# Dimev/grail-rs

Hardware: AMD Instinct MI355X
Metric: audio samples/sec (whole node) at 48 kHz, batch=65536 utterances (higher is better)
Workload: dtype f32

## Files before the change

### grail-rs_amd/csrc/api_internal.hpp

```cpp
#pragma once

#include <dlfcn.h>
#include <hip/hip_runtime.h>
#include <rccl/rccl.h>

#include <algorithm>
#include <atomic>
#include <cmath>
#include <condition_variable>
#include <cstdio>
#include <deque>
#include <map>
#include <mutex>
#include <thread>
#include <cstdlib>
#include <cstring>
#include <new>
#include <string>
#include <unordered_map>
#include <vector>

#include "../../include/grail_hip.h"
#include "kernels.h"

struct PlanCache;

#ifdef GRAIL_FAST_PROF
constexpr size_t TRUNCATED_WORDS = 8 + 64;
#else
constexpr size_t TRUNCATED_WORDS = 4;
#endif

struct grail_ctx {
    int device = 0;
    int cus = 256;
    int device_cus = 256;
    hipStream_t stream = nullptr;
    hipEvent_t ev_start = nullptr, ev_stop = nullptr;
    bool have_timing = false;
    std::vector<grail_voice> voices;
    grail::DevVoice *d_voices = nullptr;
    float *d_voice_elems = nullptr;
    struct VoiceInfo {
        bool upper_silent = false, live4_ok = false, scan_ok = false, split_ok = false;
        uint32_t warmup = 0;
    };
    std::vector<VoiceInfo> voice_info;
    bool voices_upper_silent = false;
    bool voices_live4_ok = false;
    bool voices_scan_ok = false;
    int scan_debug = 0;
    int sort_option = 1;
    int64_t pipe8_max_groups = -1;
    int64_t pipe4_max_groups = -1;
    int scan_option = 1;
    int64_t scan_max_utts = -1;
    int64_t scan_split_max = -1;
    int ragged_option = 1;
    int pipe_spread = 1;
    int two_waves_option = 1;
    int packed_option = 1;
    int composite_option = 1;
    int row_groups_option = 1;
    double voices_sharpness = INFINITY;
    std::vector<double> voice_sharpness;
    int64_t fast_limit = (int64_t)GRAIL_FAST_SHARPNESS_LIMIT;
    int mid_option = 1;
    int64_t mid_limit = (int64_t)GRAIL_FAST_SHARPNESS_LIMIT_EXACT_COEFFICIENTS;
    bool voices_split_ok = false;
    uint32_t max_warmup = 0;
    float max_rate = 0.0f;
    int split_option = 1;
    int64_t split_chunks = 0;
    int64_t split_span = 0;
    int64_t split_ff_permille = 165;
    int64_t split_min_utts = -1;
    int last_split = 0;
    int last_fast = 0;
    int last_blocks = 0;
    float max_dt = 0.0f;
    float max_pitch_jitter = 0.0f;
    int last_formants = 8, last_lanes = 0, last_pipe = 0;
    int last_packed = 0;
    uint32_t *d_truncated = nullptr;
    uint64_t slow_steps = 0;
    uint64_t fast_tiles = 0, general_steps = 0;
    uint32_t seen_counters[4] = {0, 0, 0, 0};
    int lanes_option = 0;
    int skip_silent_option = 1;
    int pipeline_option = 1;
    int pipe_round32 = 1;
    uint64_t voices_epoch = 0;
    uint64_t options_epoch = 0;
    int fast_option = 0;
    std::string last_kernel = "none";
    ncclComm_t comm = nullptr;
    uint32_t comm_rank = 0, comm_world = 1;
    void *host_pipe = nullptr;
    void *mix_state = nullptr;
};

struct grail_stream {
    const grail_batch *batch = nullptr;
    uint32_t *d_state = nullptr;
    uint64_t lanes = 0;
    int L = 1;
    bool started = false;
    bool live4 = false, half_capable = false, any_blend = false;
    uint64_t voices_epoch = 0;
    grail_batch *own = nullptr;
    uint32_t ring_cap = 0;
    uint32_t *d_counts = nullptr;
    uint32_t *d_open = nullptr;
    uint32_t *d_consumed = nullptr;
    std::vector<uint32_t> appended;
    std::vector<uint32_t> consumed;
    std::vector<uint8_t> open;
    std::vector<grail_synthesis_elem> last_elem;
    std::vector<uint8_t> last_has;
    grail::DevSeg *d_new = nullptr;
// ... 151 lines not shown
```

### grail-rs_amd/csrc/grail_api.cpp

```cpp
#include "api_internal.hpp"

using namespace grail;
using namespace grail::host;

static_assert(sizeof(grail_synthesis_elem) == 196, "SynthesisElem is 49 x f32");
static_assert(sizeof(grail_phoneme_elem) == sizeof(DevSeg), "PhonemeElem uploads as-is");
static_assert(offsetof(grail_phoneme_elem, phoneme) == offsetof(DevSeg, elem), "layout");
static_assert(offsetof(grail_phoneme_elem, frequency) == offsetof(DevSeg, frequency), "layout");
static_assert(sizeof(grail_voice) == 4 + 2 * 196 + 5 * 4, "Voice layout");
static_assert(GRAIL_UNIQUE_ID_BYTES == NCCL_UNIQUE_ID_BYTES, "unique id size");

namespace grail {
namespace host {

namespace {
thread_local std::string g_last_error;
std::atomic<uint64_t> g_epoch{0};
}

std::string &last_error() { return g_last_error; }

int fail(int status, const std::string &msg)
{
    g_last_error = msg;
// ... 426 lines not shown
        return GRAIL_OK;
    }
    if (std::strcmp(name, "skip_silent_formants") == 0) {
        ctx->skip_silent_option = value ? 1 : 0;
        return GRAIL_OK;
    }
    if (std::strcmp(name, "small_batch_pipeline") == 0) {
        ctx->pipeline_option = value ? 1 : 0;
        return GRAIL_OK;
    }
    if (std::strcmp(name, "arithmetic") == 0) {
        if (value != 0 && value != 1 && value != 2)
            return fail(GRAIL_ERR_INVALID_ARG, "arithmetic must be 0 (exact), 1 (fast) or 2 (fast, exact coefficients)");
        ctx->fast_option = (int)value;
        return GRAIL_OK;
    }
    if (std::strcmp(name, "fast_exact_coefficients") == 0) {
        ctx->mid_option = value ? 1 : 0;
        return GRAIL_OK;
    }
    if (std::strcmp(name, "fast_sharpness_limit_exact_coefficients") == 0) {
        if (value < 0) return fail(GRAIL_ERR_INVALID_ARG, "negative limit");
        ctx->mid_limit = value;
        return GRAIL_OK;
    }
    if (std::strcmp(name, "time_parallel_scan") == 0) {
        ctx->scan_option = value ? 1 : 0;
        return GRAIL_OK;
    }
    if (std::strcmp(name, "packed_launch_order") == 0) {
        ctx->packed_option = value ? 1 : 0;
        return GRAIL_OK;
    }
    if (std::strcmp(name, "sort_by_length") == 0) {
        ctx->sort_option = value ? 1 : 0;
        return GRAIL_OK;
    }
    if (std::strcmp(name, "time_split") == 0) {
        ctx->split_option = value ? 1 : 0;
        return GRAIL_OK;
    }
    if (std::strcmp(name, "time_split_chunks") == 0) {
        if (value < 0 || value > SPLIT_MAX_CHUNKS) return fail(GRAIL_ERR_INVALID_ARG, "time_split_chunks must be 0 (auto) .. 64");
        ctx->split_chunks = value;
        return GRAIL_OK;
    }
    if (std::strcmp(name, "time_split_span_samples") == 0) {
        if (value < 0 || value > 0x7fffffff) return fail(GRAIL_ERR_INVALID_ARG, "time_split_span_samples out of range");
        ctx->split_span = value;
        return GRAIL_OK;
    }
    if (std::strcmp(name, "time_split_ff_cost_permille") == 0) {
        if (value < 0 || value > 1000) return fail(GRAIL_ERR_INVALID_ARG, "time_split_ff_cost_permille must be 0 .. 1000");
        ctx->split_ff_permille = value;
        return GRAIL_OK;
    }
    if (std::strcmp(name, "time_split_min_utterances") == 0) {
        if (value < -1) return fail(GRAIL_ERR_INVALID_ARG, "negative limit");
        ctx->split_min_utts = value;
        return GRAIL_OK;
    }
    if (std::strcmp(name, "fast_sharpness_limit") == 0) {
        if (value < 0) return fail(GRAIL_ERR_INVALID_ARG, "negative limit");
        ctx->fast_limit = value;
        return GRAIL_OK;
    }
// ... 90 lines not shown
        *value = ctx->composite_option;
        return GRAIL_OK;
    }
    if (std::strcmp(name, "row_groups") == 0) {
        *value = ctx->row_groups_option;
        return GRAIL_OK;
    }
    if (std::strcmp(name, "ragged_plan") == 0) {
        *value = ctx->ragged_option;
        return GRAIL_OK;
    }
    if (std::strcmp(name, "two_waves_per_simd") == 0) {
        *value = ctx->two_waves_option;
        return GRAIL_OK;
    }
    if (std::strcmp(name, "pipeline_spread") == 0) {
        *value = ctx->pipe_spread;
        return GRAIL_OK;
    }
    if (std::strcmp(name, "pipeline4_max_groups") == 0) {
        *value = ctx->pipe4_max_groups;
        return GRAIL_OK;
    }
    if (std::strcmp(name, "pipeline8_max_groups") == 0) {
        *value = ctx->pipe8_max_groups;
        return GRAIL_OK;
    }
    if (std::strcmp(name, "pipeline_round32") == 0) {
        *value = ctx->pipe_round32;
        return GRAIL_OK;
    }
    if (std::strcmp(name, "packed_launch_order") == 0) {
        *value = ctx->packed_option;
        return GRAIL_OK;
    }
    if (std::strcmp(name, "last_launch_packed") == 0) {
        *value = ctx->last_packed;
        return GRAIL_OK;
    }
    if (std::strcmp(name, "sort_by_length") == 0) {
        *value = ctx->sort_option;
        return GRAIL_OK;
    }
    if (std::strcmp(name, "last_launch_fast") == 0) {
        *value = ctx->last_fast;
        return GRAIL_OK;
    }
    if (std::strcmp(name, "last_launch_blocks") == 0) {
        *value = ctx->last_blocks;
        return GRAIL_OK;
    }
    if (std::strcmp(name, "time_split") == 0) {
        *value = ctx->split_option;
        return GRAIL_OK;
    }
    if (std::strcmp(name, "time_split_chunks") == 0) {
        *value = ctx->split_chunks;
        return GRAIL_OK;
    }
    if (std::strcmp(name, "time_split_span_samples") == 0) {
        *value = ctx->split_span;
        return GRAIL_OK;
    }
    if (std::strcmp(name, "time_split_ff_cost_permille") == 0) {
        *value = ctx->split_ff_permille;
        return GRAIL_OK;
// ... 266 lines not shown
int grail_batch_lengths(grail_ctx *ctx, const grail_batch *batch, uint32_t max_len,
                        uint32_t *out_len)
{
    int rc = bind(ctx);
    if (rc) return rc;
    if ((rc = check_ready(ctx, batch))) return rc;
    if (!out_len && batch->n_utt) return fail(GRAIL_ERR_INVALID_ARG, "out_len is NULL");
    if (batch->n_utt == 0) return GRAIL_OK;
    uint32_t *d_len = nullptr;
    HIP_TRY(hipMalloc((void **)&d_len, (size_t)batch->n_utt * sizeof(uint32_t)));
    LenArgs a{};
    a.segs = batch->d_segs;
    a.seg_offsets = batch->d_offsets;
    a.voice_ids = batch->d_voice_ids;
    a.voices = ctx->d_voices;
    a.out_len = d_len;
    a.n_utt = batch->n_utt;
    a.n_voices = (uint32_t)ctx->voices.size();
    a.max_len = max_len;
    hipError_t e = launch_lengths(a, ctx->stream);
    if (e == hipSuccess)
        e = hipMemcpyAsync(out_len, d_len, (size_t)batch->n_utt * sizeof(uint32_t),
                           hipMemcpyDeviceToHost, ctx->stream);
    if (e == hipSuccess) e = hipStreamSynchronize(ctx->stream);
    (void)hipFree(d_len);
    if (e != hipSuccess) return hip_fail(e, "grail_batch_lengths");
    return GRAIL_OK;
}

int grail_sync(grail_ctx *ctx)
{
    int rc = bind(ctx);
    if (rc) return rc;
    uint32_t flags[4] = {0, 0, 0, 0};
    HIP_TRY(hipMemcpyAsync(flags, ctx->d_truncated, sizeof flags, hipMemcpyDeviceToHost, ctx->stream));
    HIP_TRY(hipStreamSynchronize(ctx->stream));
    const uint32_t flag = flags[0];
    ctx->slow_steps += (uint32_t)(flags[1] - ctx->seen_counters[1]);
    ctx->fast_tiles += (uint32_t)(flags[2] - ctx->seen_counters[2]);
    ctx->general_steps += (uint32_t)(flags[3] - ctx->seen_counters[3]);
    for (int i = 1; i < 4; ++i) ctx->seen_counters[i] = flags[i];
    if (flag) {
        HIP_TRY(hipMemsetAsync(ctx->d_truncated, 0, sizeof(uint32_t), ctx->stream));
        HIP_TRY(hipStreamSynchronize(ctx->stream));
    }
    if (flag) {
        return fail(GRAIL_ERR_BUFFER_TOO_SMALL,
                    "at least one utterance did not end within out_stride samples");
    }
    return GRAIL_OK;
}

const char *grail_last_kernel_name(grail_ctx *ctx) { return ctx ? ctx->last_kernel.c_str() : "none"; }

int grail_last_kernel_ms(grail_ctx *ctx, float *ms)
{
    int rc = bind(ctx);
    if (rc) return rc;
    if (!ms) return fail(GRAIL_ERR_INVALID_ARG, "ms is NULL");
    if (!ctx->have_timing) return fail(GRAIL_ERR_INVALID_ARG, "no kernel has been launched");
    HIP_TRY(hipEventSynchronize(ctx->ev_stop));
    HIP_TRY(hipEventElapsedTime(ms, ctx->ev_start, ctx->ev_stop));
    return GRAIL_OK;
}

int grail_pcm16_async(grail_ctx *ctx, const float *in_dev, uint64_t in_stride,
                      const uint32_t *len_dev, uint32_t n_utt, uint32_t max_len, int16_t *out_dev,
                      uint64_t out_stride)
{
    int rc = bind(ctx);
    if (rc) return rc;
    if (n_utt && (!in_dev || !len_dev || !out_dev)) return fail(GRAIL_ERR_INVALID_ARG, "NULL buffer");
    hipError_t e = launch_pcm16(in_dev, in_stride, len_dev, n_utt, max_len, out_dev, out_stride,
                                ctx->stream);
// ... 124 lines not shown
```

### grail-rs_amd/csrc/kernels.h

```cpp
#pragma once

#include <hip/hip_runtime.h>
#include <stdint.h>

namespace grail {

constexpr int NF = 8;
constexpr int ELEM_FLOATS = 49;
constexpr int NUM_VOICED = 2;
constexpr int PH_FIRST_VOICED = 3;
constexpr int SPLIT_MAX_CHUNKS = 64;

constexpr int F_FREQ = 1, F_BW = 9, F_SMOOTH = 17, F_BREATH = 25, F_TURB = 33, F_AMP = 41;

struct DevSeg {
    int32_t elem;
    float length;
    float blend_length;
    float frequency;
};
static_assert(sizeof(DevSeg) == 16, "DevSeg must be one dwordx4");

struct DevVoice {
    float sample_rate;
// ... 14 lines not shown
    const uint32_t *seeds;
    const uint32_t *perm;
    const float *elems;
    const DevVoice *voices;
    float *out;
    int16_t *out_pcm16;
    uint32_t *out_len;
    uint32_t *truncated;
    uint64_t out_stride;
    uint64_t cap;
    uint32_t n_utt;
    uint32_t n_voices;
    uint32_t phoneme_mode;
    uint32_t skip_silent;
    uint32_t half_capable;
    uint32_t live4;
    uint32_t pipe;
    uint32_t fast;
    uint32_t any_blend;
    uint32_t cohabit;
    const uint32_t *len_bound;
    uint32_t pipe_fill;
    uint32_t fold_from;
    uint32_t *state;
    uint64_t state_stride;
    uint32_t resume;
    uint32_t ring_cap;
    const uint32_t *seg_counts;
    const uint32_t *seg_open;
    uint32_t *seg_consumed;
    uint32_t split_chunks;
    uint32_t split_warmup;
    uint32_t split_bounds[SPLIT_MAX_CHUNKS + 1];
};

struct LenArgs {
    const DevSeg *segs;
    const uint32_t *seg_offsets;
    const uint32_t *voice_ids;
    const DevVoice *voices;
    uint32_t *out_len;
    uint32_t n_utt;
    uint32_t n_voices;
    uint32_t max_len;
};

const char *last_kernel_name();
hipError_t launch_synth(const SynthArgs &args, int lanes_per_utt, hipStream_t stream);
hipError_t launch_lengths(const LenArgs &args, hipStream_t stream);
hipError_t launch_ring_append(DevSeg *ring, float *ring_elems, uint32_t *counts, uint32_t ring_cap, const DevSeg *new_segs,
                              const float *new_elems, const uint32_t *new_offsets, uint32_t n_utt, hipStream_t stream);
hipError_t launch_scan(const SynthArgs &args, hipStream_t stream);
hipError_t launch_pcm16(const float *in, uint64_t in_stride, const uint32_t *len, uint32_t n_utt,
                        uint32_t max_len, int16_t *out, uint64_t out_stride, hipStream_t stream);
hipError_t launch_digest(const float *in, uint64_t in_stride, const uint32_t *len, uint32_t n_utt,
                         unsigned long long *sums, float *maxabs, uint32_t *nonfinite,
                         hipStream_t stream);
hipError_t launch_compare(const float *a, const float *b, uint64_t stride, const uint32_t *len_a,
                          const uint32_t *len_b, uint32_t n_utt, float *maxdiff, double *sumsq, uint32_t *bad,
                          hipStream_t stream);
uint32_t state_words(int lanes_per_utt);
uint64_t state_lanes(uint32_t n_utt, int lanes_per_utt);

namespace mix { struct MixItem; }
struct MixArgs {
    const float *rows;
// ... 15 lines not shown
```

### grail-rs_amd/csrc/synth_kernel.h

```cpp
#pragma once
#include <cstdio>
#include <type_traits>

#include "device_common.h"
#include "kernels.h"
#include "pcm16.h"

#ifndef GRAIL_MIXED_RUNS
#define GRAIL_MIXED_RUNS 1
#endif
#ifndef GRAIL_MIXED_RUNS_L1
#define GRAIL_MIXED_RUNS_L1 0
#endif
#ifndef GRAIL_MIXED_RUNS_PIPE
#define GRAIL_MIXED_RUNS_PIPE 1
#endif
#ifndef GRAIL_SPLIT_SKIP
#define GRAIL_SPLIT_SKIP 1
#endif
#ifndef GRAIL_PIPE_PARTIAL
#define GRAIL_PIPE_PARTIAL 1
#endif
#ifndef PIPE_CP8_L8
#define PIPE_CP8_L8 4
#endif
#ifndef PIPE_CP8_L4
#define PIPE_CP8_L4 2
#endif
#ifndef GRAIL_SCALAR_PACK
#define GRAIL_SCALAR_PACK 1
#endif
#ifndef GRAIL_FAST_G_SCALE
#define GRAIL_FAST_G_SCALE 262144.0f
#endif
#ifndef GRAIL_FAST_A_SCALE
#define GRAIL_FAST_A_SCALE 724.0773439350247f
#endif
#ifndef PIPE_MAX_TILES
#define PIPE_MAX_TILES 64
#endif

#ifdef GRAIL_FAST_PROF
#define PROF_ADD(k) do { const unsigned long long n_ = clock64(); prof_c[k] += n_ - prof_t0; prof_t0 = n_; } while (0)
#define PROF_CNT(k, v) do { prof_c[k] += (unsigned long long)(v); } while (0)
#else
#define PROF_ADD(k) do { } while (0)
#define PROF_CNT(k, v) do { } while (0)
#endif

namespace grail {

extern thread_local char g_kernel_name[96];

namespace {

#include "synth_kernel_parts.h"

template <int L, int T, int WAVES, int MIN_WAVES_PER_SIMD, bool STREAM, bool HALF, bool ANYBL, int NFA = NF,
          bool PIPE = false, bool FAST = false, int PQP = 2, bool SPLIT = false, bool MID = false>
__global__ __launch_bounds__(64 * WAVES, MIN_WAVES_PER_SIMD) void synth_kernel(const SynthArgs A)
{
#include "synth_kernel_state.h"

#include "synth_kernel_general_step.h"

#include "synth_kernel_calm_steps.h"

#include "synth_kernel_pipe.h"

#include "synth_kernel_scalar_packed.h"


#include "synth_kernel_fast.h"
#include "synth_kernel_flush.h"

#include "synth_kernel_fast_tile.h"

#include "synth_kernel_split.h"

#include "synth_kernel_tile_loop.h"

    if constexpr (SPLIT) {
        if (slot_used && done && !paused && n_out >= chunk_lo) {
            if (A.out_len) A.out_len[u] = n_out;
            if (truncated) atomicOr(A.truncated, 1u);
        }
    } else if (emit && j == L - 1 && slot_used) {
        if (A.out_len) A.out_len[u] = n_out;
        if (truncated) atomicOr(A.truncated, 1u);
    }
    if (streaming && A.state && slot_used && emit) {
        StateIO<false> io{A.state, A.state_stride, state_lane};
        visit_state(io);
        if constexpr (LIVE)
            if (A.ring_cap != 0u && j == L - 1 && A.seg_consumed) A.seg_consumed[u] = seg_pos;
    }
    if (emit && lane == 0 && slow_steps) atomicAdd(A.truncated + 1, slow_steps);
    if (emit && lane == 0 && fast_tiles) atomicAdd(A.truncated + 2, fast_tiles);
    if (emit && lane == 0 && general_steps) atomicAdd(A.truncated + 3, general_steps);
#ifdef GRAIL_FAST_PROF
    {
        unsigned long long *prof = reinterpret_cast<unsigned long long *>(A.truncated + 8);
        prof_c[0] = clock64() - prof_start;
        if (lane == 0) {
#pragma unroll
            for (int k = 0; k < 32; ++k)
                if (prof_c[k]) atomicAdd(prof + k, prof_c[k]);
            atomicAdd(prof + 31, 1ull);
        }
        if (prof_lane_levels) atomicAdd(prof + 17, prof_lane_levels);
    }
#endif
}

template <int L, int T, int WAVES, int MINW, bool STREAM, bool HALF, bool ANYBL, int NFA = NF, bool PIPE = false,
          bool FAST = false, int PQP = 2, bool SPLIT = false, bool MID = false>
void start(const SynthArgs &args, dim3 grid, dim3 block, hipStream_t stream)
{
    std::snprintf(g_kernel_name, sizeof g_kernel_name, "synth_kernel<L=%d,T=%d,W=%d,%d,%s%s%sNFA=%d%s%s%s%s%s>", L, T, WAVES,
                  MINW, STREAM ? "STREAM," : "", HALF ? "HALF," : "", ANYBL ? "ANYBL," : "", NFA,
                  PIPE ? ",PIPE" : "", FAST ? ",FAST" : "", PQP == 4 ? ",R16" : PQP == 8 ? ",R32" : "", SPLIT ? ",SPLIT" : "",
                  MID ? ",MID" : "");
    hipLaunchKernelGGL((synth_kernel<L, T, WAVES, MINW, STREAM, HALF, ANYBL, NFA, PIPE, FAST, PQP, SPLIT, MID>), grid, block, 0,
                       stream, args);
}

}
}
```

### grail-rs_amd/csrc/synth_kernel_parts.h

```cpp
template <int CTRL, int ROW_MASK>
__device__ __forceinline__ uint32_t umin_dpp(const uint32_t x)
{
    const uint32_t o = (uint32_t)__builtin_amdgcn_update_dpp((int)x, (int)x, CTRL, ROW_MASK, 0xF, false);
    return o < x ? o : x;
}
__device__ __forceinline__ float dpp_from_lane_below(float x)
{
    return __int_as_float(
        __builtin_amdgcn_update_dpp(0, __float_as_int(x), 0x111 , 0xF, 0xF, true));
}

__device__ __forceinline__ void wave_lds_sync()
{
    __builtin_amdgcn_fence(__ATOMIC_RELEASE, "wavefront");
    __builtin_amdgcn_wave_barrier();
    __builtin_amdgcn_fence(__ATOMIC_ACQUIRE, "wavefront");
}

template <int NV, typename V>
struct Part {
    float frequency;
    V freq[NV], bw[NV], smooth[NV], breath[NV], turb[NV], amp[NV];
};

// ... 87 lines not shown
        FOR_L { r[k] = vfma(-den[k], q[k], num[k]); r2[k] = vfma(-e_freq[k], q2[k], e_bw[k]); }
        FOR_L { g[k] = vfma(r[k], y[k], q[k]); kq[k] = vfma(r2[k], y2[k], q2[k]); }
        FOR_L d3[k] = 1.0f + g[k] * (g[k] + kq[k]);
        FOR_L y[k] = vrcp(d3[k]);
        FOR_L e[k] = vfma(-d3[k], y[k], one);
        FOR_L a1[k] = vfma(e[k], y[k], y[k]);
        constexpr int NLP = (NLIVE < NV && !KEEP_LP) ? NLIVE : NV;
#define FOR_P _Pragma("unroll") for (int k = 0; k < NLP; ++k)
        V nw[NV];
        FOR_P nw[k] = saw * (1.0f - e_breath[k]) + noise * e_breath[k];
        if constexpr (SU) {
            FOR_P st_a[k] = st_a[k] + oml_s * (nw[k] - st_a[k]);
        } else {
            V lp[NV];
            FOR_P lp[k] = exp_approx(e_smooth[k]);
            FOR_P st_a[k] = st_a[k] + (1.0f - lp[k]) * (nw[k] - st_a[k]);
        }
#undef FOR_P
        V tw[NLIVE], v0[NLIVE], a2[NLIVE], a3[NLIVE], v3[NLIVE], w1[NLIVE], w2[NLIVE];
        FOR_L tw[k] = st_a[k] * ((1.0f - e_turb[k]) + noise * e_turb[k]);
        FOR_L v0[k] = tw[k] * e_amp[k];
        FOR_L a2[k] = g[k] * a1[k];
        FOR_L a3[k] = g[k] * a2[k];
        FOR_L v3[k] = v0[k] - st_c[k];
        FOR_L w1[k] = a1[k] * st_b[k] + a2[k] * v3[k];
        FOR_L w2[k] = (st_c[k] + a2[k] * st_b[k]) + a3[k] * v3[k];
        FOR_L st_b[k] = 2.0f * w1[k] - st_b[k];
        FOR_L st_c[k] = 2.0f * w2[k] - st_c[k];
        FOR_L v1[k] = w1[k];
#pragma unroll
        for (int k = NLIVE; k < NV; ++k) v1[k] = vsplat(0.0f, st_a[0]);
    }
}
#undef FOR_L
#undef FOR_K

template <int NV, typename V>
__device__ __forceinline__ void exact_band_pass_coeffs(const V (&xf)[NV], const V (&yf)[NV], const V (&xb)[NV], const V (&yb)[NV],
                                                       const V (&ffc)[NV], const V (&ffn)[NV], const float alpha, const float oma,
                                                       const float jp, const float jomp, const float d_ffreq,
                                                       V (&a1)[NV], V (&a2)[NV], V (&a3)[NV])
{
#define FOR_K _Pragma("unroll") for (int k = 0; k < NV; ++k)
    V ef[NV], eb[NV], nff[NV], num[NV], den[NV], g[NV], kq[NV], y[NV], e[NV], q[NV], r[NV], d3[NV], y2[NV], e2[NV], q2[NV], r2[NV];
    const V one = vsplat(1.0f, xf[0]), five = vsplat(5.0f, xf[0]), m4 = vsplat(-4.0f, xf[0]);
    FOR_K ef[k] = xf[k] * oma + yf[k] * alpha;
    FOR_K eb[k] = xb[k] * oma + yb[k] * alpha;
    FOR_K nff[k] = ffc[k] * jomp + ffn[k] * jp;
    FOR_K ef[k] = ef[k] + nff[k] * d_ffreq;
    FOR_K {
        const V x = ef[k];
        const V omx = 1.0f - x, xph = x + 0.5f, hmx = 0.5f - x;
        const V ox = omx * x, ph = xph * hmx;
        num[k] = ox * vfma(m4, ph, five);
        den[k] = (xph * vfma(m4, ox, five)) * hmx;
    }
    FOR_K { y[k] = vrcp(den[k]); y2[k] = vrcp(ef[k]); }
    FOR_K { e[k] = vfma(-den[k], y[k], one); e2[k] = vfma(-ef[k], y2[k], one); }
    FOR_K { y[k] = vfma(e[k], y[k], y[k]); y2[k] = vfma(e2[k], y2[k], y2[k]); }
    FOR_K { q[k] = num[k] * y[k]; q2[k] = eb[k] * y2[k]; }
    FOR_K { r[k] = vfma(-den[k], q[k], num[k]); r2[k] = vfma(-ef[k], q2[k], eb[k]); }
    FOR_K { g[k] = vfma(r[k], y[k], q[k]); kq[k] = vfma(r2[k], y2[k], q2[k]); }
    FOR_K d3[k] = 1.0f + g[k] * (g[k] + kq[k]);
    FOR_K y[k] = vrcp(d3[k]);
    FOR_K e[k] = vfma(-d3[k], y[k], one);
    FOR_K a1[k] = vfma(e[k], y[k], y[k]);
// ... 89 lines not shown
```

### grail-rs_amd/csrc/synth_kernel_state.h

```cpp
    static_assert(!FAST || (!PIPE && !HALF), "FAST");
    static_assert(!MID || FAST, "MID is a flavour of the tolerance kernels");
    static_assert(!SPLIT || (FAST && !STREAM && L == 1 && WAVES == 1 && T == 64), "SPLIT");
    static_assert(NFA == NF || (NFA == 4 && !HALF), "NFA");
    static_assert(!PIPE || (WAVES == 4 && NFA / L == 1 && L >= 4 && !HALF && T % 4 == 0), "PIPE");
    constexpr int FPL = NFA / L;
    constexpr int W = FPL >= 2 ? 2 : 1;
    constexpr int NV = FPL / W;
    typedef typename VecOf<W>::type V;
    constexpr int S = 64 / L;
    constexpr int SP = S + 1;
    static_assert(T % 4 == 0 && (64 % (T / 4)) == 0, "T");
    if constexpr (L > 1 && !PIPE && MIN_WAVES_PER_SIMD == 1) asm volatile("" ::: "a127");

    constexpr bool FOLD_IN_FLUSH = L >= 4;
    constexpr int STAGE_FLOATS = FOLD_IN_FLUSH ? T * S * NFA : T * SP;
    __shared__ float stage_all[PIPE ? 1 : WAVES][STAGE_FLOATS];
    __shared__ uint32_t cnt_all[PIPE ? 1 : WAVES][S];
    const int wave = threadIdx.x / 64;
    float *stage = stage_all[PIPE ? 0 : wave];
    uint32_t *cnt = cnt_all[PIPE ? 0 : wave];
    const int role = PIPE ? wave : 0;
    const bool emit = !PIPE || role == 0;

    const int lane = threadIdx.x % 64;
    const int slot = lane / L;
    const int j = lane % L;
    const int f0 = j * FPL;
    const uint32_t split_groups = SPLIT ? (A.n_utt + S - 1) / S : 1u;
    const uint32_t chunk = SPLIT ? A.split_chunks - 1u - blockIdx.x / split_groups : 0u;
    uint32_t block_id = blockIdx.x;
    if constexpr (!SPLIT && !PIPE && !STREAM && MIN_WAVES_PER_SIMD == 2)
        if (A.fold_from != 0u && block_id >= A.fold_from) block_id = gridDim.x - 1u - (block_id - A.fold_from);
    const uint32_t pipe_fill = PIPE && !STREAM && A.pipe_fill != 0u ? A.pipe_fill : (uint32_t)S;
    const uint32_t u0 = SPLIT ? (blockIdx.x % split_groups) * S
                              : PIPE ? blockIdx.x * pipe_fill : (block_id * WAVES + wave) * S;
    const bool slot_used = (!PIPE || (uint32_t)slot < pipe_fill) && u0 + slot < A.n_utt;
    const uint32_t u = !slot_used ? A.n_utt : (A.perm ? A.perm[u0 + slot] : u0 + slot);
    bool done = !slot_used;
    if constexpr (SPLIT && GRAIL_SPLIT_SKIP) {
        if (A.len_bound != nullptr && slot_used && chunk > 0u && A.len_bound[u] <= A.split_bounds[chunk]) done = true;
        if (__builtin_amdgcn_ballot_w64(!done) == 0) {
#ifdef GRAIL_FAST_PROF
            if (threadIdx.x == 0) atomicAdd(reinterpret_cast<unsigned long long *>(A.truncated + 8) + 30, 1ull);
#endif
            return;
        }
    }
    const uint32_t uc = done ? 0u : u;
    __shared__ uint32_t rowid_all[PIPE ? 1 : WAVES][S];
    uint32_t *rowid = rowid_all[PIPE ? 0 : wave];
    if (A.perm && j == L - 1) rowid[slot] = uc;

    uint32_t vid = A.voice_ids ? A.voice_ids[uc] : 0u;
    if (vid >= A.n_voices) vid = 0u;
    const DevVoice VO = A.voices[vid];
// ... 190 lines not shown
```

### grail-rs_amd/csrc/synth_kernel_tile_loop.h

```cpp
    for (uint32_t base = base0;; base += T) {
        if constexpr (SPLIT) {
            if (chunk > 0u && base == reset_at) {
#pragma unroll
                for (int k = 0; k < NV; ++k) {
                    st_a[k] = vsplat(0.0f, st_a[k]);
                    st_b[k] = st_a[k];
                    st_c[k] = st_a[k];
                }
                fast_have = -1;
            }
        }
        int t = 0;
        if constexpr (FAST) {
            fast_render_tile(0);
            t = T;
        }
        constexpr bool MIXED_RUNS = GRAIL_MIXED_RUNS && !FAST && (!PIPE || GRAIL_MIXED_RUNS_PIPE) && GRAIL_SCALAR_PACK && (L > 1 || GRAIL_MIXED_RUNS_L1);
        bool mixed_shared = false, mixed_stale = false;
        uint32_t mixed_seed = 0u, mixed_sk = 0u;
        float mixed_noise = 0.0f;
        if constexpr (!FAST) PROF_ADD(8);
        while (t < T) {
            bool calm_tile = false;
            int pipe_tiles = 1;
// ... 155 lines not shown
                                }
                            } else if (ph_ >= 0) {
#pragma unroll
                                for (int q = 0; q < 2 * QP; ++q)
                                    pipe_render(ring_all[ph_ & 1][q], SPR * (ph_ % ROUNDS) + 2 * q);
                            }
                            __syncthreads();
                            if (ph_ >= 0 && ph_ % ROUNDS == ROUNDS - 1 && ph_ != all_rounds - 1) {
                                n_out += idle ? 0u : (uint32_t)T;
                                noise_seed = (uint32_t)__builtin_amdgcn_readlane((int)sk, T - 1);
                                sk = noise_seed * LCG_SKIP.mul[ahead] + LCG_SKIP.add[ahead];
                                flush_rows(base, n_out > base ? n_out - base : 0u);
                                base += T;
                            }
                        }
                        if (role == 1) {
                            hand_all[0][lane] = clk;
                            hand_all[1][lane] = jphase;
                            hand_all[2][lane] = phase;
                        }
                        __syncthreads();
                        if (role != 1) {
                            clk = hand_all[0][lane];
                            jphase = hand_all[1][lane];
                            phase = hand_all[2][lane];
                        }
                    } else if constexpr (W == 1 && NV == 1 && FOLD_IN_FLUSH) {
                        static_assert(!(W == 1 && NV == 1 && FOLD_IN_FLUSH) || (L >= 4 && T % 8 == 0), "blocks of eight, quads");
#pragma unroll 1
                        for (int tc = 0; tc < T; tc += 8) time_packed_block(tc, noise_of_lane);
                    } else if constexpr (GRAIL_SCALAR_PACK && STEPS_PER_TRIP == 2 && L >= 4 && T % 8 == 0) {
#pragma unroll 1
                        for (int tc = 0; tc < T; tc += 8) scalar_packed_block(nlive_tag, su_tag, tc, noise_of_lane);
                    } else if constexpr (GRAIL_SCALAR_PACK && STEPS_PER_TRIP == 2) {
#pragma unroll 1
                        for (int tc = 0; tc < T; tc += 2) {
                            const float nz0 = __builtin_bit_cast(
                                float, __builtin_amdgcn_readlane(__builtin_bit_cast(int, noise_of_lane), tc));
                            const float nz1 = __builtin_bit_cast(
                                float, __builtin_amdgcn_readlane(__builtin_bit_cast(int, noise_of_lane), tc + 1));
                            scalar_packed_steps(nlive_tag, su_tag, tc, nz0, nz1);
                        }
                    } else {
#pragma unroll 1
                        for (int tc = 0; tc < T; tc += STEPS_PER_TRIP) {
#pragma unroll
                            for (int h = 0; h < STEPS_PER_TRIP; ++h) {
                                const float nz = __builtin_bit_cast(
                                    float, __builtin_amdgcn_readlane(__builtin_bit_cast(int, noise_of_lane), tc + h));
                                quiet_step(nlive_tag, su_tag, std::true_type(), tc + h, clk - dt, jphase + jinc, nz);
                            }
                        }
                    }
                    t = T;
                    n_out += idle ? 0u : (uint32_t)T;
                    noise_seed = (uint32_t)__builtin_amdgcn_readlane((int)sk, T - 1);
                    return;
                }
                constexpr int RUN_STEP = L >= 4 ? 8 : 2;
                while (t < T) {
                    if constexpr (MIXED_RUNS) {
                        const bool idle_now = STREAM ? finished : done;
                        if (mixed_shared && T - t >= RUN_STEP &&
                            __builtin_amdgcn_ballot_w64(!(idle_now | (!done & quiet_ok))) == 0) {
                            const float by_clock = clk * __builtin_amdgcn_rcpf(dt) - 1.5f;
                            const float by_phase = (0.9999f - jphase) * __builtin_amdgcn_rcpf(jinc) - 0.5f;
// ... 42 lines not shown
                                                   (jphase_next > 1.0f) | (n_out >= cap32));
                    if (__builtin_expect(__builtin_amdgcn_ballot_w64(eventful) != 0, 0)) break;
                    quiet_step(nlive_tag, su_tag, std::false_type(), t, clk_next, jphase_next, 0.0f);
                    PROF_CNT(12, 1);
                    ++t;
                }
                if constexpr (MIXED_RUNS) {
                    if (mixed_stale && t >= T) {
                        const uint32_t s_ = (uint32_t)__builtin_amdgcn_readlane((int)mixed_sk, T - 1);
                        if (!done) noise_seed = s_;
                        mixed_stale = false;
                    }
                }
            };
            PROF_ADD(9);
            const bool all_su = __builtin_amdgcn_ballot_w64(!done & !smooth_uniform) == 0;
            typedef std::integral_constant<int, NV> FullTag;
            bool half = false;
            if constexpr (HALF && NV >= 2) {
                typedef std::integral_constant<int, NV / 2> HalfTag;
                half = __builtin_amdgcn_ballot_w64(!done & !upper_silent) == 0;
                if (half && all_su) quiet_run(HalfTag(), std::true_type());
                else if (half) quiet_run(HalfTag(), std::false_type());
            }
            if (!half) {
                if (all_su) quiet_run(FullTag(), std::true_type());
                else quiet_run(FullTag(), std::false_type());
            }
            if (calm_tile) { PROF_ADD(2); PROF_CNT(15, 1); PROF_CNT(16, all_su ? 1 : 0); PROF_CNT(17, half ? 1 : 0); }
            else { PROF_ADD(3); PROF_CNT(18, all_su ? 1 : 0); PROF_CNT(19, half ? 1 : 0); PROF_CNT(20, 1); }
            if (t < T) {
                ++general_steps;
                general_step(t, std::false_type());
                quiet_ok = pair_safe && (blend_pow2 || blend_div_ok);
                ++t;
                PROF_ADD(7); PROF_CNT(11, 1);
            }
        }

        const uint32_t mine = n_out > base ? n_out - base : 0u;
        constexpr int ROW_LANES = T / 4;
        constexpr int ROWS_PER_IT = 64 / ROW_LANES;
        const int rl = lane % ROW_LANES;
        const int rr = lane / ROW_LANES;
        if constexpr (SPLIT) {
            if (base < chunk_lo) {
                if (__builtin_amdgcn_ballot_w64(!done) == 0) break;
                continue;
            }
        }
        if constexpr (!FOLD_IN_FLUSH && ROWS_PER_IT <= S) {
            const bool all_full = __builtin_amdgcn_ballot_w64((j == L - 1) & (mine != (uint32_t)T)) == 0;
            constexpr bool PCM_FULL_TILE = !(L == 1 && NFA == NF);
            if (PCM_FULL_TILE && all_full && (A.out_pcm16 ? !vec16_ok : !vec_ok)) {
                wave_lds_sync();
                float w[S / ROWS_PER_IT][4];
#pragma unroll
                for (int i = 0; i < S / ROWS_PER_IT; ++i)
#pragma unroll
                    for (int q = 0; q < 4; ++q) w[i][q] = stage[(rl + q * ROW_LANES) * SP + i * ROWS_PER_IT + rr];
#pragma unroll
                for (int i = 0; i < S / ROWS_PER_IT; ++i) {
                    const uint64_t row = A.perm ? rowid[i * ROWS_PER_IT + rr] : u0 + i * ROWS_PER_IT + rr;
                    if (A.out_pcm16) {
                        int16_t *dst = A.out_pcm16 + row * A.out_stride + base + rl;
#pragma unroll
// ... 51 lines not shown
```

### grail-rs_amd/csrc/synthesize.cpp

```cpp
#include <mutex>

#include "api_internal.hpp"

using namespace grail;
using namespace grail::host;

struct PlanCache {
    uint64_t key[6];
    std::vector<Block> plan;
};

namespace grail {
namespace host {

static const uint32_t *packed_perm_of(grail_ctx *ctx, const grail_batch *root, const grail_batch *view, const Family &f,
                                      uint64_t out_stride, uint32_t slot0, uint32_t count, int *rc)
{
    *rc = GRAIL_OK;
    if (!ctx->packed_option || root->perm_host.size() < (size_t)slot0 + count) return nullptr;
    const uint32_t family = (uint32_t)f.L | f.fast << 8 | f.live4 << 16;
    static std::mutex lock;
    std::lock_guard<std::mutex> hold(lock);
    for (const PackedPerm &pp : root->packed)
        if (pp.view == view && pp.slot0 == slot0 && pp.rows == count && pp.family == family && pp.cus == (uint32_t)ctx->cus)
// ... 32 lines not shown
static int launch_block(grail_ctx *ctx, const grail_batch *root, const grail_batch *batch, const Family &f, float *out_dev,
                        int16_t *out_pcm16_dev, uint64_t out_stride, uint32_t *out_len_dev, uint32_t first, uint32_t slot0,
                        uint32_t count, bool use_perm)
{
    SynthArgs a{};
    const uint32_t row0 = use_perm ? 0u : first + slot0;
    const uint64_t out_shift = use_perm ? 0ull : (uint64_t)slot0 * out_stride;
    a.out_pcm16 = out_pcm16_dev ? out_pcm16_dev + out_shift : nullptr;
    a.segs = batch->d_segs;
    a.seg_offsets = batch->d_offsets + row0;
    a.voice_ids = batch->d_voice_ids ? batch->d_voice_ids + row0 : nullptr;
    a.seeds = batch->d_seeds ? batch->d_seeds + row0 : nullptr;
    a.perm = use_perm ? batch->d_perm + slot0 : nullptr;
    if (use_perm) {
        int rc = GRAIL_OK;
        const uint32_t *packed = packed_perm_of(ctx, root, batch, f, out_stride, slot0, count, &rc);
        if (rc) return rc;
        if (packed) {
            a.perm = packed;
            ++ctx->last_packed;
        }
    }
    a.elems = batch->phoneme_mode ? ctx->d_voice_elems : batch->d_elems;
    a.voices = ctx->d_voices;
    a.out = out_dev ? out_dev + out_shift : nullptr;
    a.out_len = out_len_dev ? out_len_dev + (use_perm ? 0u : slot0) : nullptr;
    a.truncated = ctx->d_truncated;
    a.out_stride = out_stride;
    a.cap = out_stride;
    a.n_utt = count;
    a.n_voices = (uint32_t)ctx->voices.size();
    a.phoneme_mode = batch->phoneme_mode ? 1u : 0u;
    a.skip_silent = ctx->skip_silent_option ? 1u : 0u;
    a.half_capable = batch_half_capable(ctx, batch) ? 1u : 0u;
    a.any_blend = batch->any_blend ? 1u : 0u;
    a.live4 = f.live4;
    a.fast = f.fast;
    a.cohabit = family_cohabits(ctx, f, count) ? 1u : 0u;
    a.len_bound = batch->d_len_bound && batch->len_bound_epoch == ctx->voices_epoch ? batch->d_len_bound + row0 : nullptr;
    a.pipe_fill = pipe_fill_for(ctx, batch, f, count);
    a.fold_from = 0u;
    if (a.cohabit) {
        const uint32_t waves_per_block = f.L >= 4 ? 4u : 1u, per_block = (64u / (uint32_t)f.L) * waves_per_block;
        const uint32_t blocks = (count + per_block - 1u) / per_block, round = (uint32_t)ctx_simds(ctx) / waves_per_block;
        if (blocks > round && blocks <= 2u * round) a.fold_from = round;
    }
    a.pipe = f.pipe;
    hipError_t e;
    if (f.scan) {
        a.resume = (uint32_t)ctx->scan_debug;
        a.pipe = f.scan_pipe;
        e = launch_scan(a, ctx->stream);
        ctx->last_kernel = a.live4 ? (a.pipe ? "scan_kernel<pairs=2,SPLIT,FAST>" : "scan_kernel<pairs=2,FAST>")
                                   : (a.pipe ? "scan_kernel<pairs=4,SPLIT,FAST>" : "scan_kernel<pairs=4,FAST>");
    } else {
        if (f.split_k) {
            a.split_chunks = (uint32_t)f.split_k;
            a.split_warmup = batch->phoneme_mode ? 0u : batch->elems_warmup;
            std::memcpy(a.split_bounds, f.split_bounds, sizeof a.split_bounds);
        }
        e = launch_synth(a, f.L, ctx->stream);
        ctx->last_kernel = last_kernel_name();
    }
    if (e != hipSuccess) return hip_fail(e, "synth kernel launch");
    return GRAIL_OK;
}
// ... 117 lines not shown
```

Measured before the change: 153.6 billion.

## Share per-step blend coefficients across lanes with identical phoneme pairs via LDS

Adds a shared-blend path for the L==1 scalar-packed kernel. When all live lanes in a wave share clock, dt and blend length, it groups lanes by (current, next) element key into up to 12 slots. It computes the blended formant coefficients once per key and step into an LDS table, and each lane then reads them instead of recomputing the blend per lane. This removes redundant per-lane interpolation and exp work, at the cost of extra LDS traffic, wave-level syncs, per-wave LDS allocation that can reduce occupancy, and a new filter routine. The path is enabled by default and can be switched off through an option, and a counter of shared tiles is added.

```diff
diff --git a/grail-rs_amd/csrc/api_internal.hpp b/grail-rs_amd/csrc/api_internal.hpp
--- a/grail-rs_amd/csrc/api_internal.hpp
+++ b/grail-rs_amd/csrc/api_internal.hpp
@@ -28,7 +28,7 @@
 #ifdef GRAIL_FAST_PROF
 constexpr size_t TRUNCATED_WORDS = 8 + 64;
 #else
-constexpr size_t TRUNCATED_WORDS = 4;
+constexpr size_t TRUNCATED_WORDS = 8;
 #endif
 
 struct grail_ctx {
@@ -84,8 +84,9 @@
     int last_packed = 0;
     uint32_t *d_truncated = nullptr;
     uint64_t slow_steps = 0;
-    uint64_t fast_tiles = 0, general_steps = 0;
-    uint32_t seen_counters[4] = {0, 0, 0, 0};
+    uint64_t fast_tiles = 0, general_steps = 0, shared_blend_tiles = 0;
+    uint32_t seen_counters[5] = {0, 0, 0, 0, 0};
+    int shared_blend_option = 1;
     int lanes_option = 0;
     int skip_silent_option = 1;
     int pipeline_option = 1;
diff --git a/grail-rs_amd/csrc/grail_api.cpp b/grail-rs_amd/csrc/grail_api.cpp
--- a/grail-rs_amd/csrc/grail_api.cpp
+++ b/grail-rs_amd/csrc/grail_api.cpp
@@ -482,6 +482,10 @@
         ctx->packed_option = value ? 1 : 0;
         return GRAIL_OK;
     }
+    if (std::strcmp(name, "shared_blend") == 0) {
+        ctx->shared_blend_option = value ? 1 : 0;
+        return GRAIL_OK;
+    }
     if (std::strcmp(name, "sort_by_length") == 0) {
         ctx->sort_option = value ? 1 : 0;
         return GRAIL_OK;
@@ -638,6 +642,14 @@
     }
     if (std::strcmp(name, "packed_launch_order") == 0) {
         *value = ctx->packed_option;
+        return GRAIL_OK;
+    }
+    if (std::strcmp(name, "shared_blend") == 0) {
+        *value = ctx->shared_blend_option;
+        return GRAIL_OK;
+    }
+    if (std::strcmp(name, "shared_blend_wave_tiles") == 0) {
+        *value = (int64_t)ctx->shared_blend_tiles;
         return GRAIL_OK;
     }
     if (std::strcmp(name, "last_launch_packed") == 0) {
@@ -970,14 +982,15 @@
 {
     int rc = bind(ctx);
     if (rc) return rc;
-    uint32_t flags[4] = {0, 0, 0, 0};
+    uint32_t flags[5] = {0, 0, 0, 0, 0};
     HIP_TRY(hipMemcpyAsync(flags, ctx->d_truncated, sizeof flags, hipMemcpyDeviceToHost, ctx->stream));
     HIP_TRY(hipStreamSynchronize(ctx->stream));
     const uint32_t flag = flags[0];
     ctx->slow_steps += (uint32_t)(flags[1] - ctx->seen_counters[1]);
     ctx->fast_tiles += (uint32_t)(flags[2] - ctx->seen_counters[2]);
     ctx->general_steps += (uint32_t)(flags[3] - ctx->seen_counters[3]);
-    for (int i = 1; i < 4; ++i) ctx->seen_counters[i] = flags[i];
+    ctx->shared_blend_tiles += (uint32_t)(flags[4] - ctx->seen_counters[4]);
+    for (int i = 1; i < 5; ++i) ctx->seen_counters[i] = flags[i];
     if (flag) {
         HIP_TRY(hipMemsetAsync(ctx->d_truncated, 0, sizeof(uint32_t), ctx->stream));
         HIP_TRY(hipStreamSynchronize(ctx->stream));
diff --git a/grail-rs_amd/csrc/kernels.h b/grail-rs_amd/csrc/kernels.h
--- a/grail-rs_amd/csrc/kernels.h
+++ b/grail-rs_amd/csrc/kernels.h
@@ -70,6 +70,7 @@
     uint32_t split_chunks;
     uint32_t split_warmup;
     uint32_t split_bounds[SPLIT_MAX_CHUNKS + 1];
+    uint32_t shared_blend;
 };
 
 struct LenArgs {
diff --git a/grail-rs_amd/csrc/synth_kernel.h b/grail-rs_amd/csrc/synth_kernel.h
--- a/grail-rs_amd/csrc/synth_kernel.h
+++ b/grail-rs_amd/csrc/synth_kernel.h
@@ -26,6 +26,9 @@
 #endif
 #ifndef PIPE_CP8_L4
 #define PIPE_CP8_L4 2
+#endif
+#ifndef GRAIL_SHARED_BLEND
+#define GRAIL_SHARED_BLEND 1
 #endif
 #ifndef GRAIL_SCALAR_PACK
 #define GRAIL_SCALAR_PACK 1
@@ -78,6 +81,8 @@
 
 #include "synth_kernel_split.h"
 
+#include "synth_kernel_shared_blend.h"
+
 #include "synth_kernel_tile_loop.h"
 
     if constexpr (SPLIT) {
@@ -98,6 +103,8 @@
     if (emit && lane == 0 && slow_steps) atomicAdd(A.truncated + 1, slow_steps);
     if (emit && lane == 0 && fast_tiles) atomicAdd(A.truncated + 2, fast_tiles);
     if (emit && lane == 0 && general_steps) atomicAdd(A.truncated + 3, general_steps);
+    if constexpr (SHARED_BLEND)
+        if (lane == 0 && sb_tiles) atomicAdd(A.truncated + 4, sb_tiles);
 #ifdef GRAIL_FAST_PROF
     {
         unsigned long long *prof = reinterpret_cast<unsigned long long *>(A.truncated + 8);
diff --git a/grail-rs_amd/csrc/synth_kernel_parts.h b/grail-rs_amd/csrc/synth_kernel_parts.h
--- a/grail-rs_amd/csrc/synth_kernel_parts.h
+++ b/grail-rs_amd/csrc/synth_kernel_parts.h
@@ -143,6 +143,51 @@
         for (int k = NLIVE; k < NV; ++k) v1[k] = vsplat(0.0f, st_a[0]);
     }
 }
+
+template <int NV, typename V>
+__device__ __forceinline__ void formant_filters_shared(const float saw, const float oml_s, const V (&e_freq)[NV],
+                                                       const V (&e_bw)[NV], const V (&omb)[NV], const V (&nb)[NV],
+                                                       const V (&tf)[NV], const V (&e_amp)[NV], V (&st_a)[NV],
+                                                       V (&st_b)[NV], V (&st_c)[NV], V (&v1)[NV])
+{
+    V num[NV], den[NV], g[NV], kq[NV], a1[NV], y[NV], e[NV], q[NV], r[NV], d3[NV], y2[NV], e2[NV], q2[NV], r2[NV];
+    const V one = vsplat(1.0f, st_a[0]);
+    const V five = vsplat(5.0f, st_a[0]);
+    const V m4 = vsplat(-4.0f, st_a[0]);
+    FOR_K {
+        const V x = e_freq[k];
+        const V omx = 1.0f - x;
+        const V xph = x + 0.5f;
+        const V hmx = 0.5f - x;
+        const V ox = omx * x;
+        const V ph = xph * hmx;
+        num[k] = ox * vfma(m4, ph, five);
+        den[k] = (xph * vfma(m4, ox, five)) * hmx;
+    }
+    FOR_K { y[k] = vrcp(den[k]); y2[k] = vrcp(e_freq[k]); }
+    FOR_K { e[k] = vfma(-den[k], y[k], one); e2[k] = vfma(-e_freq[k], y2[k], one); }
+    FOR_K { y[k] = vfma(e[k], y[k], y[k]); y2[k] = vfma(e2[k], y2[k], y2[k]); }
+    FOR_K { q[k] = num[k] * y[k]; q2[k] = e_bw[k] * y2[k]; }
+    FOR_K { r[k] = vfma(-den[k], q[k], num[k]); r2[k] = vfma(-e_freq[k], q2[k], e_bw[k]); }
+    FOR_K { g[k] = vfma(r[k], y[k], q[k]); kq[k] = vfma(r2[k], y2[k], q2[k]); }
+    FOR_K d3[k] = 1.0f + g[k] * (g[k] + kq[k]);
+    FOR_K y[k] = vrcp(d3[k]);
+    FOR_K e[k] = vfma(-d3[k], y[k], one);
+    FOR_K a1[k] = vfma(e[k], y[k], y[k]);
+    V nw[NV], tw[NV], v0[NV], a2[NV], a3[NV], v3[NV], w1[NV], w2[NV];
+    FOR_K nw[k] = saw * omb[k] + nb[k];
+    FOR_K st_a[k] = st_a[k] + oml_s * (nw[k] - st_a[k]);
+    FOR_K tw[k] = st_a[k] * tf[k];
+    FOR_K v0[k] = tw[k] * e_amp[k];
+    FOR_K a2[k] = g[k] * a1[k];
+    FOR_K a3[k] = g[k] * a2[k];
+    FOR_K v3[k] = v0[k] - st_c[k];
+    FOR_K w1[k] = a1[k] * st_b[k] + a2[k] * v3[k];
+    FOR_K w2[k] = (st_c[k] + a2[k] * st_b[k]) + a3[k] * v3[k];
+    FOR_K st_b[k] = 2.0f * w1[k] - st_b[k];
+    FOR_K st_c[k] = 2.0f * w2[k] - st_c[k];
+    FOR_K v1[k] = w1[k];
+}
 #undef FOR_L
 #undef FOR_K
 
diff --git a/grail-rs_amd/csrc/synth_kernel_shared_blend.h b/grail-rs_amd/csrc/synth_kernel_shared_blend.h
--- /dev/null
+++ b/grail-rs_amd/csrc/synth_kernel_shared_blend.h
@@ -0,0 +1,230 @@
+    typedef float f4 __attribute__((ext_vector_type(4)));
+    auto sb_f4 = [](const float a, const float b, const float c, const float d) __attribute__((always_inline)) {
+        f4 q;
+        q.x = a; q.y = b; q.z = c; q.w = d;
+        return q;
+    };
+    auto shared_blend_slots = [&](const uint64_t busy) __attribute__((always_inline)) {
+        if constexpr (SHARED_BLEND) {
+            const int kc = cur.elem >= 0 ? cur.elem : -1;
+            const int kn = (nxt.some && nxt.elem >= 0) ? nxt.elem : -1;
+            uint64_t todo = busy;
+            int n = 0;
+            bool rep = false;
+            sb_slot = 0;
+#pragma unroll 1
+            while (todo != 0 && n < SB_P) {
+                const int l = __builtin_ctzll(todo);
+                const int c0 = __builtin_amdgcn_readlane(kc, l), n0 = __builtin_amdgcn_readlane(kn, l);
+                const bool mine = !done & (kc == c0) & (kn == n0);
+                sb_slot = mine ? n : sb_slot;
+                rep = rep | (lane == l);
+                todo &= ~__builtin_amdgcn_ballot_w64(mine);
+                ++n;
+            }
+            sb_nkeys = todo == 0 ? n : 0;
+            if (sb_nkeys != 0 && rep) {
+                f4 *row = reinterpret_cast<f4 *>(sb_rows + sb_slot * SB_ROW);
+                auto put = [&](const int at, const V(&f)[NV]) __attribute__((always_inline)) {
+                    row[at] = sb_f4(vget(f[0], 0), vget(f[0], 1), vget(f[1], 0), vget(f[1], 1));
+                };
+                put(0, X.freq); put(1, X.bw); put(2, X.breath); put(3, X.turb); put(4, X.amp);
+                put(5, Y.freq); put(6, Y.bw); put(7, Y.breath); put(8, Y.turb); put(9, Y.amp);
+                row[10] = sb_f4(vget(X.smooth[0], 0), vget(Y.smooth[0], 0), silent_pair ? 1.0f : 0.0f, 0.0f);
+            }
+            wave_lds_sync();
+        }
+    };
+    auto shared_blend_engages = [&]() __attribute__((always_inline)) -> bool {
+        if constexpr (SHARED_BLEND) {
+            if (A.shared_blend == 0u) return false;
+            const uint64_t busy = __builtin_amdgcn_ballot_w64(!done);
+            if (busy == 0) return false;
+            if (sb_dirty) {
+                sb_dirty = false;
+                shared_blend_slots(busy);
+            }
+            if (sb_nkeys == 0) return false;
+            const int first = __builtin_ctzll(busy);
+            const int c0 = __builtin_amdgcn_readlane(__builtin_bit_cast(int, clk), first);
+            const int d0 = __builtin_amdgcn_readlane(__builtin_bit_cast(int, dt), first);
+            const int b0 = __builtin_amdgcn_readlane(__builtin_bit_cast(int, blend_length), first);
+            const bool same = done | ((__builtin_bit_cast(int, clk) == c0) & (__builtin_bit_cast(int, dt) == d0) &
+                                      (__builtin_bit_cast(int, blend_length) == b0));
+            return __builtin_amdgcn_ballot_w64(!same) == 0;
+        } else {
+            return false;
+        }
+    };
+    struct SbEntry {
+        f4 omb, nb, freq, bw, tf, amp;
+        float oml;
+    };
+    auto sb_read = [&](SbEntry &e, const int step) __attribute__((always_inline)) {
+        const f4 *p = reinterpret_cast<const f4 *>(sb_table + (step * SB_P + sb_slot) * SB_STRIDE);
+        e.omb = p[0]; e.nb = p[1]; e.freq = p[2]; e.bw = p[3]; e.tf = p[4]; e.amp = p[5];
+        e.oml = reinterpret_cast<const float *>(p)[27];
+    };
+    auto sb_read_alpha = [&](const int step) __attribute__((always_inline)) {
+        return *reinterpret_cast<const f2 *>(sb_table + (step * SB_P + sb_slot) * SB_STRIDE + 24);
+    };
+    auto sb_v = [](V &lo, V &hi, const f4 q) __attribute__((always_inline)) {
+        vset(lo, 0, q.x); vset(lo, 1, q.y); vset(hi, 0, q.z); vset(hi, 1, q.w);
+    };
+    auto shared_blend_steps = [&](const int t0, const float noise_of_lane, float &clk_u, const float dt_u, const float bl_u,
+                                  const float ibl_u, const bool pow2_u) __attribute__((always_inline)) {
+        if constexpr (SHARED_BLEND) {
+            static_assert(NV == 2 && W == 2 && L == 1 && SB_STEPS == 16 && T % SB_STEPS == 0, "lanes = 4 pairs x 16 steps");
+            const int s = lane & (SB_STEPS - 1);
+            float clk_s = clk_u;
+#pragma unroll
+            for (int i = 0; i < SB_STEPS; ++i) {
+                clk_u = clk_u - dt_u;
+                clk_s = i == s ? clk_u : clk_s;
+            }
+            float ratio = clk_s * ibl_u;
+            if constexpr (ANYBL) {
+                const float rem = vfma(-bl_u, ratio, clk_s);
+                const float quot = vfma(rem, ibl_u, ratio);
+                ratio = pow2_u ? ratio : quot;
+            }
+            const float alpha_s = __builtin_fminf(ratio, 1.0f);
+            const float nz = __builtin_bit_cast(
+                float, __builtin_amdgcn_ds_bpermute((t0 + s) * 4, __builtin_bit_cast(int, noise_of_lane)));
+            wave_lds_sync();
+#pragma unroll 1
+            for (int k0 = 0; k0 < sb_nkeys; k0 += 64 / SB_STEPS) {
+                const int key = k0 + lane / SB_STEPS;
+                const f4 *row = reinterpret_cast<const f4 *>(sb_rows + key * SB_ROW);
+                V xf[NV], xw[NV], xb[NV], xt[NV], xa[NV], yf[NV], yw[NV], yb[NV], yt[NV], ya[NV];
+                sb_v(xf[0], xf[1], row[0]); sb_v(xw[0], xw[1], row[1]); sb_v(xb[0], xb[1], row[2]);
+                sb_v(xt[0], xt[1], row[3]); sb_v(xa[0], xa[1], row[4]);
+                sb_v(yf[0], yf[1], row[5]); sb_v(yw[0], yw[1], row[6]); sb_v(yb[0], yb[1], row[7]);
+                sb_v(yt[0], yt[1], row[8]); sb_v(ya[0], ya[1], row[9]);
+                const f4 sm = row[10];
+                const float a = sm.z != 0.0f ? 1.0f : alpha_s;
+                const float om = 1.0f - a;
+                V e_breath[NV], e_freq[NV], e_bw[NV], e_turb[NV], e_amp[NV], omb[NV], nb[NV], tf[NV];
+#pragma unroll
+                for (int k = 0; k < NV; ++k) {
+                    e_breath[k] = xb[k] * om + yb[k] * a;
+                    e_freq[k] = xf[k] * om + yf[k] * a;
+                    e_bw[k] = xw[k] * om + yw[k] * a;
+                    e_turb[k] = xt[k] * om + yt[k] * a;
+                    e_amp[k] = xa[k] * om + ya[k] * a;
+                    omb[k] = 1.0f - e_breath[k];
+                    nb[k] = nz * e_breath[k];
+                    tf[k] = (1.0f - e_turb[k]) + nz * e_turb[k];
+                }
+                const float es = sm.x * om + sm.y * a;
+                const float oml = 1.0f - exp_approx(es);
+                f4 *e = reinterpret_cast<f4 *>(sb_table + (s * SB_P + key) * SB_STRIDE);
+                e[0] = sb_f4(vget(omb[0], 0), vget(omb[0], 1), vget(omb[1], 0), vget(omb[1], 1));
+                e[1] = sb_f4(vget(nb[0], 0), vget(nb[0], 1), vget(nb[1], 0), vget(nb[1], 1));
+                e[2] = sb_f4(vget(e_freq[0], 0), vget(e_freq[0], 1), vget(e_freq[1], 0), vget(e_freq[1], 1));
+                e[3] = sb_f4(vget(e_bw[0], 0), vget(e_bw[0], 1), vget(e_bw[1], 0), vget(e_bw[1], 1));
+                e[4] = sb_f4(vget(tf[0], 0), vget(tf[0], 1), vget(tf[1], 0), vget(tf[1], 1));
+                e[5] = sb_f4(vget(e_amp[0], 0), vget(e_amp[0], 1), vget(e_amp[1], 0), vget(e_amp[1], 1));
+                e[6] = sb_f4(a, om, 0.0f, oml);
+            }
+            wave_lds_sync();
+            SbEntry E0, E1;
+            f2 AO0 = sb_read_alpha(0), AO1 = sb_read_alpha(1);
+            __builtin_amdgcn_sched_barrier(0);
+            sb_read(E0, 0);
+            __builtin_amdgcn_sched_barrier(0);
+            sb_read(E1, 1);
+            __builtin_amdgcn_sched_barrier(0);
+#pragma unroll 1
+            for (int tc = 0; tc < SB_STEPS; tc += 2) {
+                const f2 one2 = vsplat(1.0f, f2());
+                const float clk0 = clk - dt, clk1 = clk0 - dt;
+                const float jp0 = jphase + jinc, jp1 = jp0 + jinc;
+                clk = clk1;
+                jphase = jp1;
+                f2 JP, alpha, oma;
+                JP.x = jp0; JP.y = jp1;
+                alpha.x = AO0.x; alpha.y = AO1.x;
+                oma.x = AO0.y; oma.y = AO1.y;
+                const f2 jomp = 1.0f - JP;
+                f2 frequency = X.frequency * oma + Y.frequency * alpha;
+                __builtin_amdgcn_sched_barrier(0);
+                AO0 = sb_read_alpha((tc + 2) & (SB_STEPS - 1));
+                AO1 = sb_read_alpha((tc + 3) & (SB_STEPS - 1));
+                __builtin_amdgcn_sched_barrier(0);
+                const f2 n_freq = fn_cur * jomp + fn_next * JP;
+                frequency = frequency + n_freq * d_freq;
+                const f2 omf = 1.0f - frequency;
+                const float ph0 = phase;
+                const bool head0 = ph0 < frequency.x, tail0 = ph0 > omf.x;
+                const float ph1 = __builtin_amdgcn_fractf(ph0 + frequency.x);
+                const bool head1 = ph1 < frequency.y, tail1 = ph1 > omf.y;
+                phase = __builtin_amdgcn_fractf(ph1 + frequency.y);
+                f2 PH;
+                PH.x = ph0; PH.y = ph1;
+                const f2 phm1 = PH - 1.0f;
+                f2 dividend;
+                dividend.x = head0 ? ph0 : phm1.x;
+                dividend.y = head1 ? ph1 : phm1.y;
+                const f2 tt = div_exact<true>(dividend, frequency);
+                const f2 tt2 = tt * tt;
+                f2 s_tt2, sgn, polyblep;
+                s_tt2.x = __uint_as_float(__float_as_uint(tt2.x) ^ (head0 ? 0x80000000u : 0u));
+                s_tt2.y = __uint_as_float(__float_as_uint(tt2.y) ^ (head1 ? 0x80000000u : 0u));
+                sgn.x = head0 ? -1.0f : 1.0f;
+                sgn.y = head1 ? -1.0f : 1.0f;
+                const f2 pb = vfma(vsplat(2.0f, f2()), tt, s_tt2) + sgn;
+                polyblep.x = (head0 | tail0) ? pb.x : 0.0f;
+                polyblep.y = (head1 | tail1) ? pb.y : 0.0f;
+                const f2 saw2 = vfma(vsplat(2.0f, f2()), PH, -one2) - polyblep;
+                V F_omb[2][NV], F_nb[2][NV], F_freq[2][NV], F_bw[2][NV], F_tf[2][NV], F_amp[2][NV];
+#pragma unroll
+                for (int h = 0; h < 2; ++h) {
+                    const SbEntry E = h == 0 ? E0 : E1;
+                    const float jp = vget(JP, h), jm = vget(jomp, h);
+                    sb_v(F_omb[h][0], F_omb[h][1], E.omb); sb_v(F_nb[h][0], F_nb[h][1], E.nb);
+                    sb_v(F_freq[h][0], F_freq[h][1], E.freq); sb_v(F_bw[h][0], F_bw[h][1], E.bw);
+                    sb_v(F_tf[h][0], F_tf[h][1], E.tf); sb_v(F_amp[h][0], F_amp[h][1], E.amp);
+#pragma unroll
+                    for (int k = 0; k < NV; ++k) {
+                        const V n_ff = ff_cur[k] * jm + ff_next[k] * jp;
+                        const V n_fa = fa_cur[k] * jm + fa_next[k] * jp;
+                        F_freq[h][k] = F_freq[h][k] + n_ff * d_ffreq;
+                        const V delta = (n_fa + 1.0f) * amp_scale;
+                        const V mul = 1.0f - delta;
+                        F_amp[h][k] = F_amp[h][k] * mul;
+                    }
+                }
+#pragma unroll
+                for (int h = 0; h < 2; ++h) {
+                    V v1[NV];
+                    formant_filters_shared<NV, V>(vget(saw2, h), h == 0 ? E0.oml : E1.oml, F_freq[h], F_bw[h], F_omb[h],
+                                                  F_nb[h], F_tf[h], F_amp[h], st_a, st_b, st_c, v1);
+                    float run = 0.0f;
+#pragma unroll
+                    for (int k = 0; k < NV; ++k)
+#pragma unroll
+                        for (int c = 0; c < W; ++c) run = run + vget(v1[k], c);
+                    if (NFA < NF) run = run + 0.0f;
+                    stage[(t0 + tc + h) * SP + slot] = run * 0.5f;
+                    __builtin_amdgcn_sched_barrier(0);
+                    sb_read(h == 0 ? E0 : E1, (tc + 2 + h) & (SB_STEPS - 1));
+                    __builtin_amdgcn_sched_barrier(0);
+                }
+            }
+        }
+    };
+    auto shared_blend_tile = [&](const float noise_of_lane) __attribute__((always_inline)) {
+        if constexpr (SHARED_BLEND) {
+            const int first = __builtin_ctzll(__builtin_amdgcn_ballot_w64(!done));
+            float clk_u = __builtin_bit_cast(float, __builtin_amdgcn_readlane(__builtin_bit_cast(int, clk), first));
+            const float dt_u = __builtin_bit_cast(float, __builtin_amdgcn_readlane(__builtin_bit_cast(int, dt), first));
+            const float bl_u = __builtin_bit_cast(float, __builtin_amdgcn_readlane(__builtin_bit_cast(int, blend_length), first));
+            const float ibl_u =
+                __builtin_bit_cast(float, __builtin_amdgcn_readlane(__builtin_bit_cast(int, inv_blend_length), first));
+            const bool pow2_u = __builtin_amdgcn_readlane(blend_pow2 ? 1 : 0, first) != 0;
+#pragma unroll 1
+            for (int t0 = 0; t0 < T; t0 += SB_STEPS) shared_blend_steps(t0, noise_of_lane, clk_u, dt_u, bl_u, ibl_u, pow2_u);
+            ++sb_tiles;
+        }
+    };
diff --git a/grail-rs_amd/csrc/synth_kernel_state.h b/grail-rs_amd/csrc/synth_kernel_state.h
--- a/grail-rs_amd/csrc/synth_kernel_state.h
+++ b/grail-rs_amd/csrc/synth_kernel_state.h
@@ -21,6 +21,20 @@
     uint32_t *cnt = cnt_all[PIPE ? 0 : wave];
     const int role = PIPE ? wave : 0;
     const bool emit = !PIPE || role == 0;
+
+    constexpr bool SHARED_BLEND = GRAIL_SHARED_BLEND && L == 1 && !STREAM && !FAST && !PIPE && NFA == 4 && GRAIL_SCALAR_PACK;
+    constexpr int SB_P = 12, SB_STEPS = 16, SB_STRIDE = 28, SB_ROW = 44;
+    float *sb_table = nullptr, *sb_rows = nullptr;
+    if constexpr (SHARED_BLEND) {
+        __shared__ __attribute__((aligned(16))) float sb_table_all[WAVES][SB_STEPS * SB_P * SB_STRIDE];
+        __shared__ __attribute__((aligned(16))) float sb_rows_all[WAVES][SB_P * SB_ROW];
+        sb_table = sb_table_all[wave];
+        sb_rows = sb_rows_all[wave];
+    }
+    int sb_slot = 0;
+    int sb_nkeys = 0;
+    bool sb_dirty = true;
+    uint32_t sb_tiles = 0;
 
     const int lane = threadIdx.x % 64;
     const int slot = lane / L;
diff --git a/grail-rs_amd/csrc/synth_kernel_tile_loop.h b/grail-rs_amd/csrc/synth_kernel_tile_loop.h
--- a/grail-rs_amd/csrc/synth_kernel_tile_loop.h
+++ b/grail-rs_amd/csrc/synth_kernel_tile_loop.h
@@ -211,6 +211,20 @@
                     } else if constexpr (GRAIL_SCALAR_PACK && STEPS_PER_TRIP == 2 && L >= 4 && T % 8 == 0) {
 #pragma unroll 1
                         for (int tc = 0; tc < T; tc += 8) scalar_packed_block(nlive_tag, su_tag, tc, noise_of_lane);
+                    } else if constexpr (SHARED_BLEND && STEPS_PER_TRIP == 2 && decltype(su_tag)::value &&
+                                         decltype(nlive_tag)::value == NV) {
+                        if (shared_blend_engages()) {
+                            shared_blend_tile(noise_of_lane);
+                        } else {
+#pragma unroll 1
+                            for (int tc = 0; tc < T; tc += 2) {
+                                const float nz0 = __builtin_bit_cast(
+                                    float, __builtin_amdgcn_readlane(__builtin_bit_cast(int, noise_of_lane), tc));
+                                const float nz1 = __builtin_bit_cast(
+                                    float, __builtin_amdgcn_readlane(__builtin_bit_cast(int, noise_of_lane), tc + 1));
+                                scalar_packed_steps(nlive_tag, su_tag, tc, nz0, nz1);
+                            }
+                        }
                     } else if constexpr (GRAIL_SCALAR_PACK && STEPS_PER_TRIP == 2) {
 #pragma unroll 1
                         for (int tc = 0; tc < T; tc += 2) {
@@ -319,6 +333,7 @@
             if (t < T) {
                 ++general_steps;
                 general_step(t, std::false_type());
+                if constexpr (SHARED_BLEND) sb_dirty = true;
                 quiet_ok = pair_safe && (blend_pow2 || blend_div_ok);
                 ++t;
                 PROF_ADD(7); PROF_CNT(11, 1);
diff --git a/grail-rs_amd/csrc/synthesize.cpp b/grail-rs_amd/csrc/synthesize.cpp
--- a/grail-rs_amd/csrc/synthesize.cpp
+++ b/grail-rs_amd/csrc/synthesize.cpp
@@ -88,6 +88,7 @@
     a.n_voices = (uint32_t)ctx->voices.size();
     a.phoneme_mode = batch->phoneme_mode ? 1u : 0u;
     a.skip_silent = ctx->skip_silent_option ? 1u : 0u;
+    a.shared_blend = ctx->shared_blend_option ? 1u : 0u;
     a.half_capable = batch_half_capable(ctx, batch) ? 1u : 0u;
     a.any_blend = batch->any_blend ? 1u : 0u;
     a.live4 = f.live4;
```

Result: slower. 141.1 billion (median of 2 runs) (-8.2%).
